# see--/speech_recognition

Measured on AMD Instinct MI355X. Metric: 1s 16kHz clips/sec training throughput, higher is better.
Workload: dtype f32; 1 GPU; configs[1]: 12-class conv_1d_time_sliced_with_attention, batch 1024/GPU synthetic 16000-sample fp32 clips, sampler+augment+STFT/mel(80,60)+raw fwd/bwd+RMSprop; global_batch=1024, parallelism=dp1, clip_bank=65536

## Files before the change

speech_recognition_amd/csrc/bn.hip:

```cpp
#include "internal.h"

namespace {

constexpr int FIN_CG = 16, FIN_RG = 16;
#ifndef KWS_FIN_U
#define KWS_FIN_U 16
#endif
constexpr int FIN_U = KWS_FIN_U;

__device__ float g_zero_fin[8] = {0.f, 0.f, 0.f, 0.f, 0.f, 0.f, 0.f, 0.f};

__global__ __launch_bounds__(256) void bn_stats_finalize_kernel(const float* __restrict__ part, int n_tiles,
                                                                double inv_count, int C,
                                                                const float* __restrict__ gamma,
                                                                const float* __restrict__ beta, float eps,
                                                                float one_minus_momentum, float* moving_mean,
                                                                float* moving_var, float* __restrict__ bn) {
  __shared__ double red[2][FIN_RG][FIN_CG];
  const int cg = threadIdx.x % FIN_CG, rg = threadIdx.x / FIN_CG;
  const int c = blockIdx.x * FIN_CG + cg;
  double s = 0.0, ss = 0.0;
  if (c < C) {
    for (int t = rg; t < n_tiles; t += FIN_U * FIN_RG) {
      float a[FIN_U], b[FIN_U];
// ... 22 lines not shown
      ss += red[1][r][cg];
    }
    const double mean = s * inv_count;
    double var = ss * inv_count - mean * mean;
    if (var < 0.0) var = 0.0;
    const float rstd = (float)(1.0 / sqrt(var + (double)eps));
    const float meanf = (float)mean, varf = (float)var;
    const float scale = gamma[c] * rstd;
    bn[c] = scale;
    bn[C + c] = beta[c] - meanf * scale;
    bn[2 * C + c] = meanf;
    bn[3 * C + c] = rstd;
    if (moving_mean) {
      moving_mean[c] = moving_mean[c] - (moving_mean[c] - meanf) * one_minus_momentum;
      moving_var[c] = moving_var[c] - (moving_var[c] - varf) * one_minus_momentum;
    }
  }
}

__global__ __launch_bounds__(256) void slice_reduce_kernel(const float* __restrict__ in, float* __restrict__ out,
                                                           int n, int W, int rows_per) {
  const int w = blockIdx.x * 256 + threadIdx.x;
  const int s = blockIdx.y;
  if (w >= W) return;
  const int r0 = s * rows_per;
  int r1 = r0 + rows_per;
  if (r1 > n) r1 = n;
  float a0 = 0.f, a1 = 0.f, a2 = 0.f, a3 = 0.f;
  int r = r0;
  for (; r + 3 < r1; r += 4) {
// ... 178 lines not shown
int pre_reduce(const float* part, int n, int W, float* scratch, hipStream_t st, const float** out_part, int* out_n) {
  if (scratch == nullptr || n <= KWS_PRE_REDUCE_MIN) {
    *out_part = part;
    *out_n = n;
    return KWS_OK;
  }
  const int rows_per = ceil_div(n, KWS_REDUCE_SLICES);
  const int S = ceil_div(n, rows_per);
  hipLaunchKernelGGL(slice_reduce_kernel, dim3((unsigned)ceil_div(W, 256), (unsigned)S), dim3(256), 0, st, part, scratch,
                     n, W, rows_per);
  KWS_LAUNCH_CHECK("slice_reduce_kernel");
  *out_part = scratch;
  *out_n = S;
  return KWS_OK;
}

}

int kws_dw_grad_finalize_batch(const float* const* part, const int* n_parts, const int* C, float* const* dw, int count,
                               hipStream_t stream) {
  KWS_REQUIRE(part && n_parts && C && dw && count > 0 && count <= KWS_DW_FIN_BATCH, "dw_grad_finalize_batch: bad arguments (count=%d)", count);
  DwFinBatch b;
  int blocks = 0;
  double bytes = 0;
  for (int i = 0; i < count; ++i) {
    KWS_REQUIRE(part[i] && dw[i] && n_parts[i] > 0 && n_parts[i] <= 8 * KWS_REDUCE_SLICES && C[i] > 0,
                "dw_grad_finalize_batch: bad entry %d (rows %d)", i, n_parts[i]);
    b.part[i] = part[i]; b.dw[i] = dw[i]; b.n_parts[i] = n_parts[i]; b.C[i] = C[i];
    blocks += ceil_div(C[i], FIN_CG);
    b.blk_end[i] = blocks;
// ... 7 lines not shown
}

extern "C" {

int kws_bn_stats_finalize(const float* stats_part, int n_tiles, int64_t count, int C, const float* gamma,
                          const float* beta, float eps, float momentum, float* moving_mean, float* moving_var,
                          float* bn, float* scratch, void* stream) {
  KWS_REQUIRE(stats_part && gamma && beta && bn, "bn_stats_finalize: NULL pointer");
  KWS_REQUIRE(n_tiles > 0 && count > 0 && C > 0, "bn_stats_finalize: bad sizes");
  KWS_REQUIRE((moving_mean == nullptr) == (moving_var == nullptr), "bn_stats_finalize: moving stats must both be set");
  const float omm = (float)(1.0 - (double)momentum);
  KwsProfScope prof("bn_finalize", 0.0, 8.0 * n_tiles * C, (hipStream_t)stream);
#ifdef KWS_ABL_NO_FIN
  return KWS_OK;
#endif
  KWS_TRY(pre_reduce(stats_part, n_tiles, 2 * C, scratch, (hipStream_t)stream, &stats_part, &n_tiles));
  hipLaunchKernelGGL(bn_stats_finalize_kernel, dim3((unsigned)ceil_div(C, FIN_CG)), dim3(FIN_CG * FIN_RG), 0, (hipStream_t)stream,
                     stats_part, n_tiles, 1.0 / (double)count, C, gamma, beta, eps, omm, moving_mean, moving_var, bn);
  KWS_LAUNCH_CHECK("bn_stats_finalize_kernel");
  return KWS_OK;
}

int kws_bn_infer_prepare(const float* gamma, const float* beta, const float* moving_mean, const float* moving_var,
                         float eps, int C, float* bn, void* stream) {
  KWS_REQUIRE(gamma && beta && moving_mean && moving_var && bn && C > 0, "bn_infer_prepare: bad arguments");
  hipLaunchKernelGGL(bn_infer_prepare_kernel, dim3((unsigned)ceil_div(C, 256)), dim3(256), 0, (hipStream_t)stream,
                     gamma, beta, moving_mean, moving_var, eps, C, bn);
  KWS_LAUNCH_CHECK("bn_infer_prepare_kernel");
  return KWS_OK;
}
// ... 59 lines not shown
```

speech_recognition_amd/csrc/conv1.hip:

```cpp
#include "internal.h"

#ifndef KWS_C1_WS
#define KWS_C1_WS 0
#endif
#ifndef KWS_C1_ABL
#define KWS_C1_ABL 0
#endif

namespace {

typedef float f32x16 __attribute__((ext_vector_type(16)));

constexpr int NOUT = 128;
constexpr int FM = 64;
constexpr int UM = 32;
#ifndef KWS_C1W_OCC
#define KWS_C1W_OCC 3
#endif
#ifndef KWS_C1W_ABL
#define KWS_C1W_ABL 0
#endif

struct Conv1Args {
  const float* x;
// ... 470 lines not shown
__global__ __launch_bounds__(256, KWS_C1W_OCC) void conv1_wgrad_slabsum_kernel(Conv1Args p, SlabBatch b, int n_conv) {
  __shared__ float sA[2][UM * KF];
  __shared__ float4 red[4][64];
  if ((int)blockIdx.x < n_conv) conv1_wgrad_body<KF>(p, sA, blockIdx.x);
  else kws_reduce_slabs_batch_body(b, (int)blockIdx.x - n_conv, red);
}

__global__ __launch_bounds__(256) void conv1_unfold_sum_kernel(const float* __restrict__ ws, float* __restrict__ dW,
                                                               int groups, int64_t group_stride, int taps, int cin, int hop) {
  const int i = blockIdx.x * 256 + threadIdx.x;
  if (i >= taps * cin * (NOUT / 4)) return;
  const int n4 = i % (NOUT / 4), jc = i / (NOUT / 4);
  const int j = jc / cin, c = jc - j * cin;
  const float4* src = reinterpret_cast<const float4*>(ws) + (int64_t)(hop * j + c) * (NOUT / 4) + n4;
  float4 s = make_float4(0.f, 0.f, 0.f, 0.f);
  for (int g = 0; g < groups; ++g) {
    const float4 v = src[(int64_t)g * group_stride];
    s.x += v.x; s.y += v.y; s.z += v.z; s.w += v.w;
  }
  reinterpret_cast<float4*>(dW)[i] = s;
}

struct WgradPlan {
  int S;
  int64_t chunk;
};
WgradPlan wgrad_plan(int64_t M) {
  WgradPlan pl;
  int64_t chunk = ceil_div64(ceil_div64(M, 256 * KWS_C1W_OCC), UM) * UM;
  if (chunk < UM) chunk = UM;
  pl.chunk = chunk;
  pl.S = (int)ceil_div64(M, chunk);
  return pl;
// ... 77 lines not shown
```

speech_recognition_amd/csrc/gemm.hip:

```cpp
#include "common.h"
#include "internal.h"

#include <algorithm>
#include <map>
#include <mutex>
#include <tuple>
#include <type_traits>

typedef float f32x16 __attribute__((ext_vector_type(16)));

#ifdef KWS_GEMM_STAMP
__device__ unsigned long long g_stamps[8192][8];
extern "C" __attribute__((visibility("default"))) int kws_debug_read_stamps(unsigned long long* out) {
  return (int)hipMemcpyFromSymbol(out, HIP_SYMBOL(g_stamps), sizeof(g_stamps));
}
#endif

namespace {

constexpr int NXCD = 8;

struct NNArgs {
  const float* A;
  const float* W;
// ... 1117 lines not shown
__global__ __launch_bounds__(256) void transpose_kernel(const float* in, float* out, int rows, int cols) {
  __shared__ float tile[32][33];
  const int bx = blockIdx.x * 32, by = blockIdx.y * 32;
  const int tx = threadIdx.x & 31, ty = threadIdx.x >> 5;
  for (int r = ty; r < 32; r += 8) {
    const int y = by + r, x = bx + tx;
    tile[r][tx] = (y < rows && x < cols) ? in[(int64_t)y * cols + x] : 0.f;
  }
  __syncthreads();
  for (int r = ty; r < 32; r += 8) {
    const int y = bx + r, x = by + tx;
    if (y < cols && x < rows) out[(int64_t)y * rows + x] = tile[tx][r];
  }
}

struct TransposeBatch {
  const float* in[KWS_TRANSPOSE_BATCH];
  float* out[KWS_TRANSPOSE_BATCH];
  int rows[KWS_TRANSPOSE_BATCH], cols[KWS_TRANSPOSE_BATCH], tile_end[KWS_TRANSPOSE_BATCH];
  int n;
};
__global__ __launch_bounds__(256) void transpose_batch_kernel(TransposeBatch b) {
  __shared__ float tile[32][33];
  int m = 0;
  while (m + 1 < b.n && (int)blockIdx.x >= b.tile_end[m]) ++m;
  const int t = blockIdx.x - (m ? b.tile_end[m - 1] : 0);
  const int rows = b.rows[m], cols = b.cols[m];
  const int tx_n = (cols + 31) / 32;
  const int bx = (t % tx_n) * 32, by = (t / tx_n) * 32;
  const float* in = b.in[m];
  float* out = b.out[m];
  const int tx = threadIdx.x & 31, ty = threadIdx.x >> 5;
  for (int r = ty; r < 32; r += 8) {
    const int y = by + r, x = bx + tx;
    tile[r][tx] = (y < rows && x < cols) ? in[(int64_t)y * cols + x] : 0.f;
  }
  __syncthreads();
  for (int r = ty; r < 32; r += 8) {
    const int y = bx + r, x = by + tx;
    if (y < cols && x < rows) out[(int64_t)y * rows + x] = tile[tx][r];
  }
}

__global__ __launch_bounds__(256) void reduce_slabs_batch_kernel(SlabBatch b) {
  __shared__ float4 red[4][64];
  kws_reduce_slabs_batch_body(b, blockIdx.x, red);
}

struct TNPlan {
  int bko, bno;
  int k_tiles, n_tiles, S;
  int64_t chunk;
};
bool tn_ws_eligible(int K, int N, bool gather) { return !gather && K % 64 == 0 && N % 64 == 0; }
#ifndef KWS_TN_MAX_S
#define KWS_TN_MAX_S 256
// ... 433 lines not shown
  const unsigned gx = (unsigned)ceil_div64(n4, 64);
  if (S > 128 && gx < 256) {
    const int per_group = 32, groups = ceil_div(S, per_group);
    hipLaunchKernelGGL(reduce_slabs_kernel, dim3(gx, (unsigned)groups), dim3(256), 0, st, ws, const_cast<float*>(ws), n4, S,
                       n4, per_group, (int64_t)per_group * n4);
    KWS_LAUNCH_CHECK("reduce_slabs_kernel");
    hipLaunchKernelGGL(reduce_slabs_kernel, dim3(gx), dim3(256), 0, st, ws, out, n4, groups, (int64_t)per_group * n4, 0,
                       (int64_t)0);
  } else {
    hipLaunchKernelGGL(reduce_slabs_kernel, dim3(gx), dim3(256), 0, st, ws, out, n4, S, (int64_t)-1, 0, (int64_t)0);
  }
  KWS_LAUNCH_CHECK("reduce_slabs_kernel");
  return KWS_OK;
}

int kws_transpose_batch_f32(const float* const* in, float* const* out, const int* rows, const int* cols, int n,
                            hipStream_t stream) {
  KWS_REQUIRE(in && out && rows && cols && n > 0 && n <= KWS_TRANSPOSE_BATCH, "transpose_batch: bad arguments (n=%d)", n);
  TransposeBatch b;
  int tiles = 0;
  double bytes = 0;
  for (int i = 0; i < n; ++i) {
    KWS_REQUIRE(in[i] && out[i] && rows[i] > 0 && cols[i] > 0, "transpose_batch: bad matrix %d", i);
    b.in[i] = in[i]; b.out[i] = out[i]; b.rows[i] = rows[i]; b.cols[i] = cols[i];
    tiles += ceil_div(rows[i], 32) * ceil_div(cols[i], 32);
    b.tile_end[i] = tiles;
    bytes += 8.0 * rows[i] * cols[i];
  }
  b.n = n;
  KwsProfScope prof("transpose", 0.0, bytes, stream);
  hipLaunchKernelGGL(transpose_batch_kernel, dim3((unsigned)tiles), dim3(256), 0, stream, b);
  KWS_LAUNCH_CHECK("transpose_batch_kernel");
  return KWS_OK;
}

}
```

speech_recognition_amd/csrc/internal.h:

```cpp
#pragma once
#include "common.h"

struct kws_ts_tail_args {
  const float* y; const float* bn; const float* W1; const float* b1; const float* W2; const float* labels;
  float* probs; float* g; float* part; float* xd; float* fd; float* dl1; float* dl2; float* per_loss;
  float* per_correct; float* att; int B, T, C, NC; uint64_t seed; uint32_t step; float keep_prob; float label_smoothing;
  int loss_batch; int64_t row_offset; int train;
};
int kws_ts_tail_launch(const kws_ts_tail_args* p, hipStream_t st);
constexpr int KWS_SMALL_WGRAD_SLICES = 32;
int kws_small_wgrad_launch(const float* X, const float* D, float* out, float* out_bias, int B, int K, int N,
                           float* scratch, hipStream_t st);
int kws_metrics_launch(const float* per_loss, const float* per_correct, int B, float* metrics, hipStream_t st);
struct kws_tail_post_args {
  const float* X2; const float* D2; float* ws2; int K2, N2;
  const float* X1; const float* D1; float* ws1; int K1, N1;
  float* bias1;
  const float* per_loss; const float* per_correct; float* metrics;
  int B;
};
int kws_tail_post_launch(const kws_tail_post_args* a, int* S_out, hipStream_t st);
bool kws_conv1_supported(const kws_gather_t* g, const kws_gather_t* unfolded, int N);
int kws_conv1_stats_rows(int64_t M);
int kws_conv1_fwd(const float* x, const kws_gather_t* g, const kws_gather_t* unfolded, const float* W, float* y, int B, int N,
                  float* stats, hipStream_t st);
int64_t kws_conv1_wgrad_workspace_floats(int64_t M);
int kws_conv1_wgrad(const float* x, const kws_gather_t* g, const kws_gather_t* unfolded, const float* G, float* dW, int B,
                    int N, float* workspace, hipStream_t st);
int kws_conv1_wgrad_slabs(const float* x, const kws_gather_t* g, const kws_gather_t* unfolded, const float* G, float* dW, int B,
                          int N, float* workspace, const float* const* sl_ws, float* const* sl_out, const int64_t* sl_n,
                          const int* sl_S, int n_sl, hipStream_t st);
extern "C" int kws_reduce_slab_groups_f32(float* ws, int64_t n, int S, int per_group, hipStream_t st);
extern "C" int kws_reduce_slabs_f32(const float* ws, float* out, int64_t n, int S, hipStream_t st);
extern "C" int kws_dwconv_bwd_acc_f32(const float* dz, const float* y, const float* w, const float* add, float* g, float* part,
                                      int B, int L_in, int L_out, int C, int stride, int pad_l, hipStream_t st);
extern "C" int kws_dwconv_bwd_acc_strided_f32(const float* dz, const float* y, const float* w, const float* add, int add_stride, int add_len,
// ... 44 lines not shown
int kws_gbn_bwd_finish(float* g, const float* y, const float* bn, int64_t M, const kws_gbn_cols* c, const float* part, int rows,
                       float* coef, float* dgamma0, int64_t pstride, int64_t boff, hipStream_t st);
struct kws_flat_tail_args {
  const float* y; const float* bn; int Ng;
  const float* Wd; const float* bd; const float* labels;
  float* probs; float* fd; float* dl; float* dA; float* per_loss; float* per_correct;
  int B, D, F, NC;
  uint64_t seed; uint32_t step; float keep_prob; int loss_batch; int64_t row_offset; uint32_t layer_id;
  int raw;
};
int kws_flat_tail_launch(const kws_flat_tail_args* a, int training, hipStream_t st);
int kws_pool3s2_same_fwd_pitch(const float* y, const float* bn, float* z, int zp, int B, int L, int C, hipStream_t st);
int kws_pool3s2_same_bwd_pitch(const float* dz, int zp, const float* y, const float* bn, float* g, float* part, int B, int L, int C,
                               hipStream_t st);
#ifdef __HIPCC__
__device__ __forceinline__ void kws_add4(float4& a, const float4 b) { a.x += b.x; a.y += b.y; a.z += b.z; a.w += b.w; }
__device__ __forceinline__ void kws_reduce_slabs_batch_body(const SlabBatch& b, int bid, float4 (*red)[64]) {
  int m = 0;
  while (m + 1 < b.n && bid >= b.blk_end[m]) ++m;
  const int t = bid - (m ? b.blk_end[m - 1] : 0);
  const int col = threadIdx.x & 63, grp = threadIdx.x >> 6;
  const int64_t n4 = b.n4[m];
  const int S = b.S[m];
  const int64_t i = (int64_t)t * 64 + col;
  const float4* w = reinterpret_cast<const float4*>(b.ws[m]);
  float4 s0 = make_float4(0.f, 0.f, 0.f, 0.f), s1 = s0, s2 = s0, s3 = s0;
  if (i < n4 && b.order[m]) {
    float4 t2 = s0;
    int k = grp;
    for (; k + 4 < S; k += 8) {
// ... 108 lines not shown
      used += need;
      ++count;
      return 0;
    }
    const int rc2 = kws_gemm_nn_f32(dY, WT, dZ, M, cout, cin, nullptr, st);
    if (rc2) return rc2;
    return gemm(Z, dY, dW, M, cin, cout, st);
  }
};
constexpr int KWS_DW_FIN_BATCH = 16;
int kws_dw_grad_finalize_batch(const float* const* part, const int* n_parts, const int* C, float* const* dw, int count,
                               hipStream_t stream);
constexpr int KWS_BN_INFER_BATCH = 16;
extern "C" int kws_bn_infer_prepare_batch(const float* const* gamma, const float* const* beta, const float* const* mm, const float* const* mv,
                               float eps, const int* C, float* const* bn, int count, hipStream_t stream);
constexpr int KWS_TRANSPOSE_BATCH = 16;
extern "C" int kws_transpose_batch_f32(const float* const* in, float* const* out, const int* rows, const int* cols, int n,
                                       hipStream_t stream);

struct kws_stft_plan {
  int frame_len, frame_step, fft_len, n_bins, n_mel, n_out;
  float log_offset, log_floor;
  int n_w;
  float* window;
  float2* w256;
  float2* w512;
  int* band_start;
  int* band_cnt;
  int* band_ofs;
  float* band_w;
  float* dct;
  float* dct64;
  float* b4;
// ... 14 lines not shown
```

speech_recognition_amd/csrc/net.hip:

```cpp
#include "net_internal.h"
#include <math.h>
#include <stdlib.h>

int64_t kws_net_add_tensor(kws_net* n, const std::string& name, std::vector<int64_t> shape, bool is_state, float l2,
                           int fan_in, int fan_out, float init) {
  kws_tensor_info_t t;
  memset(&t, 0, sizeof(t));
  snprintf(t.name, sizeof(t.name), "%s", name.c_str());
  int64_t size = 1;
  t.ndim = (int)shape.size();
  for (int i = 0; i < t.ndim; ++i) {
    t.shape[i] = shape[i];
    size *= shape[i];
  }
  t.size = size;
  t.is_state = is_state ? 1 : 0;
  t.l2 = l2;
  t.fan_in = fan_in;
  t.fan_out = fan_out;
  t.init = init;
  int64_t& cursor = is_state ? n->n_state : n->n_params;
  t.offset = cursor;
  cursor += (size + 3) / 4 * 4;
  n->tensors.push_back(t);
// ... 326 lines not shown
  float* red = ws + lo.red;
  const Dw3Run r{&lo.a, params, state, grads, ws, B, red, part, coef, DZ, st};
  const bool conv1_direct = kws_conv1_supported(&gather1f, &gather1, C1);
  const bool run_head = phase != 2;
  const int gmode = kws_net_get_gemm_mode(net);
  const bool h2 = gmode == 2;
  auto w_slots = [&](int i) { return slots(lo, ws, 0, i); };
  auto z_slots = [&](int i) { return slots(lo, ws, 1, i); };
  auto g_slots = [&](int i) { return slots(lo, ws, 2, i); };
  float* Gb[2] = {ws + lo.G, ws + lo.G2};
  KwsSlabQueue q;
  q.base = ws + lo.tns;
  q.cap = lo.tns_cap;
  q.allow_pair = gmode == 0;
  KWS_REQUIRE(nb + 2 <= KWS_SLAB_BATCH, "net: %d blocks exceed the slab batch", nb);
  if (run_head) {
    KWS_HIP(hipMemsetAsync(grads, 0, (size_t)net->n_params * 4, st));
    if (h2) KWS_TRY(split_kernels(lo, params, ws, true, st));
    {
      const int64_t M = (int64_t)B * lad.L1;
      const BnRef& bn1 = lad.bn1;
      if (conv1_direct) {
        KWS_TRY(kws_conv1_fwd(x, &gather1f, &gather1, params + conv1, r.y(0), B, C1, part, st));
      } else {
        KWS_TRY(fold_conv1(params, ws + lo.w1f, st));
        KWS_TRY(kws_gemm_gather_f32(x, &gather1f, ws + lo.w1f, r.y(0), B, C1, part, st));
      }
      const int rows1 = conv1_direct ? kws_conv1_stats_rows(M) : kws_gemm_gather_stats_rows(M);
      KWS_TRY(kws_bn_stats_finalize(part, rows1, M, C1, params + bn1.gamma, params + bn1.beta, KWS_BN_EPS, KWS_BN_MOMENTUM,
                                    state + bn1.mm, state + bn1.mv, r.bn_at(0), red, st));
    }
    KWS_TRY(blocks_fwd(lo, r, h2, part));
    kws_ts_tail_args t;
    memset(&t, 0, sizeof(t));
    t.y = r.y(nb); t.bn = r.bn_at(nb); t.W1 = params + d1k; t.b1 = params + d1b;
    t.W2 = params + d2k; t.labels = y_onehot; t.probs = probs; t.g = Gb[nb % 2]; t.part = part; t.xd = ws + lo.xd;
    t.fd = ws + lo.fd; t.dl1 = ws + lo.dl1; t.dl2 = ws + lo.dl2; t.per_loss = ws + lo.per_loss;
    t.per_correct = ws + lo.per_correct; t.att = ws + lo.att; t.B = B; t.T = T; t.C = C; t.NC = NC; t.seed = seed;
    t.step = step; t.keep_prob = DROP_KEEP; t.label_smoothing = LABEL_SMOOTH; t.loss_batch = loss_batch;
    t.row_offset = row_offset; t.train = 1;
    KWS_TRY(kws_ts_tail_launch(&t, st));
    bool tail_fused = false;
    if (gmode == 0) {
      kws_tail_post_args tp;
      tp.X2 = t.fd; tp.D2 = t.dl2; tp.ws2 = ws + lo.swg; tp.K2 = 2 * C; tp.N2 = NC;
      tp.X1 = t.xd; tp.D1 = t.dl1; tp.ws1 = ws + lo.swg1; tp.K1 = T * C; tp.N1 = T;
      tp.bias1 = grads + d1b; tp.per_loss = t.per_loss; tp.per_correct = t.per_correct; tp.metrics = metrics; tp.B = B;
      int S_tail = 0;
      const int rc = kws_tail_post_launch(&tp, &S_tail, st);
      if (rc < 0) return rc;
      tail_fused = rc == 0;
      if (tail_fused && S_tail > 0) {
        KWS_TRY(q.push(ws + lo.swg, grads + d2k, (int64_t)2 * C * NC, -S_tail, st));
        KWS_TRY(q.push(ws + lo.swg1, grads + d1k, (int64_t)T * C * T, -S_tail, st));
      }
    }
    if (!tail_fused) {
      KWS_TRY(kws_metrics_launch(t.per_loss, t.per_correct, B, metrics, st));
      KWS_TRY(kws_small_wgrad_launch(t.fd, t.dl2, grads + d2k, nullptr, B, 2 * C, NC, ws + lo.swg, st));
      KWS_TRY(kws_small_wgrad_launch(t.xd, t.dl1, grads + d1k, grads + d1b, B, T * C, T, ws + lo.swg, st));
    }
    const BnRef& last = lad.blocks[nb - 1].bn;
    KWS_TRY(kws_dw_bwd_finalize(part, B, (int64_t)B * T, last.C, nullptr, grads + last.gamma, grads + last.beta, coef, red, st));
    KWS_TRY(lad.transpose_all(r));
  }
  const int i_hi = phase == 2 ? split - 1 : nb - 1, i_lo = phase == 1 ? split : 0;
  for (int i = i_hi; i >= i_lo; --i) {
    const Dw3Block& b = lad.blocks[i];
    const int64_t M = (int64_t)B * b.Lout;
    float* Gcur = Gb[(i + 1) % 2];
    if (i == nb - 1)
      KWS_TRY(kws_bn_bwd_apply_amax(Gcur, r.y(i + 1), r.bn_at(i + 1), params + b.bn.gamma, coef, M, b.cout, h2 ? g_slots(i) : nullptr, st));
    if (!h2) {
      KWS_TRY(q.pair(Gcur, r.WT(i), DZ, r.z(i), grads + b.pw, M, b.cin, b.cout, st));
    } else {
      if (kws_gemm_nn_f16x2_supported(M, b.cout, b.cin))
        KWS_TRY(kws_gemm_nn_f16x2_f32(Gcur, ws + lo.WPd[i], DZ, M, b.cout, b.cin, g_slots(i), w_slots(i), nullptr, st));
      else
        KWS_TRY(kws_gemm_nn_f32(Gcur, r.WT(i), DZ, M, b.cout, b.cin, nullptr, st));
// ... 147 lines not shown
```

speech_recognition_amd/csrc/net_dw3ladder.hip:

```cpp
#include "net_internal.h"

int Dw3Ladder::build(KerasNames& kn, const int (*spec)[2], int n, int fm, int input_size) {
  int L = L1, cin = C1;
  for (int i = 0; i < n; ++i) {
    Dw3Block b;
    b.stride = spec[i][0];
    b.cin = cin;
    b.cout = spec[i][1] * fm;
    b.Lin = L;
    if (b.stride == 2) {
      kws_same_pad(L, 3, 2, &b.Lout, &b.pad_l);
    } else {
      b.Lout = L - 2;
      b.pad_l = 0;
    }
    KWS_REQUIRE(b.Lout >= 1, "net: input_size %d is too short: block %d keeps no row", input_size, i);
    b.dw = kn.dw(cin);
    b.pw = kn.conv(1, cin, b.cout, KWS_L2_COEF);
    b.bn = kn.bn(b.cout);
    blocks.push_back(b);
    L = b.Lout;
    cin = b.cout;
  }
  return KWS_OK;
// ... 60 lines not shown
  return KWS_OK;
}

int Dw3Ladder::infer_tables(const Dw3Run& r) const {
  KWS_REQUIRE(nb() + 1 <= KWS_BN_INFER_BATCH, "net: %d blocks exceed the BatchNorm table batch", nb());
  const float *ga[KWS_BN_INFER_BATCH], *be[KWS_BN_INFER_BATCH], *mm[KWS_BN_INFER_BATCH], *mv[KWS_BN_INFER_BATCH];
  float* tb[KWS_BN_INFER_BATCH];
  int Cs[KWS_BN_INFER_BATCH];
  for (int l = 0; l <= nb(); ++l) {
    const BnRef& b = l == 0 ? bn1 : blocks[l - 1].bn;
    ga[l] = r.params + b.gamma; be[l] = r.params + b.beta; mm[l] = r.state + b.mm; mv[l] = r.state + b.mv; tb[l] = r.bn_at(l); Cs[l] = b.C;
  }
  return kws_bn_infer_prepare_batch(ga, be, mm, mv, KWS_BN_EPS, Cs, tb, nb() + 1, r.st);
}

int Dw3Ladder::transpose_all(const Dw3Run& r) const {
  KWS_REQUIRE(nb() <= KWS_TRANSPOSE_BATCH, "net: %d blocks exceed the transpose batch", nb());
  const float* tin[KWS_TRANSPOSE_BATCH];
  float* tout[KWS_TRANSPOSE_BATCH];
  int trows[KWS_TRANSPOSE_BATCH], tcols[KWS_TRANSPOSE_BATCH];
  for (int i = 0; i < nb(); ++i) {
    tin[i] = r.params + blocks[i].pw; tout[i] = r.WT(i);
    trows[i] = blocks[i].cin; tcols[i] = blocks[i].cout;
  }
  return kws_transpose_batch_f32(tin, tout, trows, tcols, nb(), r.st);
}

int Dw3Ladder::fwd_dw(int i, const Dw3Run& r, unsigned* amax) const {
  const Dw3Block& b = blocks[i];
  return kws_dwconv_fwd_amax_f32(r.y(i), r.bn_at(i), r.params + b.dw, r.z(i), r.B, b.Lin, b.Lout, b.cin, b.stride, b.pad_l, amax, r.st);
}

int Dw3Ladder::stats_finalize(int i, const Dw3Run& r, const float* stats, int rows) const {
  const Dw3Block& b = blocks[i];
  return kws_bn_stats_finalize(stats, rows, (int64_t)r.B * b.Lout, b.cout, r.params + b.bn.gamma, r.params + b.bn.beta, KWS_BN_EPS,
                               KWS_BN_MOMENTUM, r.state + b.bn.mm, r.state + b.bn.mv, r.bn_at(i + 1), r.red, r.st);
}

int Dw3Ladder::fwd_block_f32(int i, const Dw3Run& r, float* stats, unsigned* amax) const {
  const Dw3Block& b = blocks[i];
  const int64_t M = (int64_t)r.B * b.Lout;
// ... 17 lines not shown
```

speech_recognition_amd/csrc/net_internal.h:

```cpp
#pragma once
#include <string.h>

#include <algorithm>
#include <atomic>
#include <memory>
#include <string>
#include <vector>

#include "internal.h"

constexpr float KWS_BN_EPS = 1e-3f;
constexpr float KWS_BN_MOMENTUM = 0.99f;
constexpr float KWS_L2_COEF = 1e-5f;

struct BnRef {
  int64_t gamma, beta;
  int64_t mm, mv;
  int C;
};
inline kws_gbn_refs kws_gbn_layer_refs(const BnRef& r, const float* params, float* state) {
  return kws_gbn_refs{params + r.gamma, 0, r.beta - r.gamma, state + r.mm, 0, r.mv - r.mm};
}
inline int kws_gbn_layer_bwd(float* dA, const float* y, const float* bn, const float* add, int64_t M, const kws_gbn_cols& c, float* part,
                             float* coef, float* grads, const BnRef& r, hipStream_t st) {
// ... 192 lines not shown
  float* bn_at(int l) const { return ws + o->bn + o->bn_stride * l; }
};
struct Dw3Ladder {
  int L1 = 0, C1 = 0;
  BnRef bn1;
  std::vector<Dw3Block> blocks;
  int nb() const { return (int)blocks.size(); }
  int build(KerasNames& kn, const int (*spec)[2], int n, int fm, int input_size);
  Dw3Sizes sizes(int B) const;
  void take_acts(Bump& bp, int B, bool training, const Dw3Sizes& s, Dw3Offsets* o) const;
  void take_bn(Bump& bp, int maxC, Dw3Offsets* o) const;
  void take_WT(Bump& bp, Dw3Offsets* o) const;
  int debug_view(const Dw3Offsets& o, int B, int what, int index, int64_t* offset_floats, int64_t* count) const;
  int infer_tables(const Dw3Run& r) const;
  int transpose_all(const Dw3Run& r) const;
  int fwd_dw(int i, const Dw3Run& r, unsigned* amax) const;
  int stats_finalize(int i, const Dw3Run& r, const float* stats, int rows) const;
  int fwd_block_f32(int i, const Dw3Run& r, float* stats, unsigned* amax) const;
  int bwd_block_input(int i, const Dw3Run& r, float* dy, unsigned* amax) const;
};

int kws_block_out_fwd(const float* y, const float* bn, const float* res, const float* res_bn, float* o, int B,
                      int L, int C, int pool, hipStream_t st);
int kws_block_out_dw_fwd(const float* y, const float* bn, const float* res, const float* res_bn, const float* w, float* o, float* z, int B,
                         int L, int C, int pool, hipStream_t st);
int kws_block_join_bwd_parts(int B, int L, int C, int pool);
int kws_block_join_bwd(const float* dO, const float* y, const float* bn, const float* gamma, const float* coef, float* out,
                       float* part, int pass, int B, int L, int C, int pool, int relu, hipStream_t st);
int64_t kws_block_out_bwd_part_floats(int B, int L, int C, int pool);
int kws_block_out_bwd(const float* dO, const float* y, const float* bn, float* g, float* part, int B, int L, int C,
// ... 49 lines not shown
```

speech_recognition_amd/csrc/tail.hip:

```cpp
#include "internal.h"

namespace {

constexpr int MAXT = 16;
constexpr int MAXNC = 64;

struct TailArgs {
  const float* y;
  const float* bn;
  const float* W1;
  const float* b1;
  const float* W2;
  const float* labels;
  float* probs;
  float* g;
  float* part;
  float* xd;
  float* fd;
  float* dl1;
  float* dl2;
  float* per_loss;
  float* per_correct;
  float* att_out;
  int B, T, C, NC;
// ... 517 lines not shown
  }
  if (threadIdx.x == 0) {
    metrics[0] = (float)rl[0];
    metrics[1] = rc[0];
    metrics[2] = 0.f;
    metrics[3] = 0.f;
  }
}
__global__ __launch_bounds__(256) void metrics_kernel(const float* per_loss, const float* per_correct, int B,
                                                      float* metrics) {
  metrics_body(per_loss, per_correct, B, metrics);
}

struct TailPost {
  kws_tail_post_args a;
  int rows_per, S, gx2, gx1;
};
__global__ __launch_bounds__(256) void tail_post_kernel(TailPost p) {
  int b = blockIdx.x;
  if (b < p.gx2 * p.S) {
    small_wgrad_rows_body<16>(p.a.X2, p.a.D2, p.a.ws2, p.a.B, p.a.K2, p.a.N2, p.rows_per, b % p.gx2, b / p.gx2);
    return;
  }
  b -= p.gx2 * p.S;
  if (b < p.gx1 * p.S) {
    small_wgrad_rows_body<16>(p.a.X1, p.a.D1, p.a.ws1, p.a.B, p.a.K1, p.a.N1, p.rows_per, b % p.gx1, b / p.gx1);
    return;
  }
  b -= p.gx1 * p.S;
  if (b == 0) metrics_body(p.a.per_loss, p.a.per_correct, p.a.B, p.a.metrics);
  else colsum_body<16, 256>(p.a.D1, p.a.bias1, p.a.B, p.a.N1);
}

}

int kws_ts_tail_launch(const kws_ts_tail_args* p, hipStream_t st) {
  KWS_REQUIRE(p->T > 0 && p->T <= MAXT && p->NC > 0 && p->NC <= MAXNC && p->C > 0, "ts_tail: bad shape T=%d NC=%d",
              p->T, p->NC);
  const int TC = p->T * p->C;
  const size_t lds_floats = (size_t)TC + 4 * p->C + 4 * MAXNC + 4 * MAXT + 3 * MAXNC + 256 + MAXNC + MAXT;
  KWS_REQUIRE(lds_floats * 4 <= 160 * 1024, "ts_tail: T*C=%d does not fit LDS", TC);
  TailArgs a{};
  a.y = p->y; a.bn = p->bn; a.W1 = p->W1; a.b1 = p->b1; a.W2 = p->W2; a.labels = p->labels; a.probs = p->probs;
  a.g = p->g; a.part = p->part; a.xd = p->xd; a.fd = p->fd; a.dl1 = p->dl1; a.dl2 = p->dl2;
  a.per_loss = p->per_loss; a.per_correct = p->per_correct; a.att_out = p->att;
  a.B = p->B; a.T = p->T; a.C = p->C; a.NC = p->NC;
// ... 46 lines not shown
      KWS_TRY(kws_reduce_slabs_f32(scratch, out, n, S, st));
    } else {
      hipLaunchKernelGGL(slab_sum_kernel, dim3((unsigned)ceil_div64(n, 256)), dim3(256), 0, st, scratch, out, n, S);
      KWS_LAUNCH_CHECK("slab_sum_kernel");
    }
  }
  if (out_bias) {
    if (N <= 16) hipLaunchKernelGGL((colsum_kernel<16, 256>), dim3(1), dim3(256), 0, st, D, out_bias, B, N);
    else if (N <= 32) hipLaunchKernelGGL((colsum_kernel<32, 1024>), dim3(1), dim3(1024), 0, st, D, out_bias, B, N);
    else hipLaunchKernelGGL((colsum_kernel<64, 1024>), dim3(1), dim3(1024), 0, st, D, out_bias, B, N);
    KWS_LAUNCH_CHECK("colsum_kernel");
  }
  return KWS_OK;
}

int kws_tail_post_launch(const kws_tail_post_args* a, int* S_out, hipStream_t st) {
  KWS_REQUIRE(a && S_out && a->X2 && a->D2 && a->ws2 && a->X1 && a->D1 && a->ws1 && a->per_loss && a->per_correct && a->metrics && a->B > 0,
              "tail_post: bad arguments");
  int S = KWS_SMALL_WGRAD_SLICES;
  if (S > a->B) S = a->B;
  const int rows_per = ceil_div(a->B, S);
  S = ceil_div(a->B, rows_per);
  if (S <= 1 || a->N1 > 16 || a->N2 > 16 || rows_per > KWS_SMALL_WGRAD_ROWS || ((int64_t)a->K1 * a->N1) % 4 != 0 ||
      ((int64_t)a->K2 * a->N2) % 4 != 0)
    return 1;
  TailPost p;
  p.a = *a; p.rows_per = rows_per; p.S = S; p.gx2 = ceil_div(a->K2, 256); p.gx1 = ceil_div(a->K1, 256);
  const int blocks = (p.gx2 + p.gx1) * S + 1 + (a->bias1 ? 1 : 0);
  KwsProfScope prof("small_wgrad", 2.0 * a->B * ((double)a->K1 * a->N1 + (double)a->K2 * a->N2),
                    4.0 * ((double)a->B * (a->K1 + a->K2 + a->N1 + a->N2) + (double)S * ((double)a->K1 * a->N1 + (double)a->K2 * a->N2)), st);
  hipLaunchKernelGGL(tail_post_kernel, dim3((unsigned)blocks), dim3(256), 0, st, p);
  KWS_LAUNCH_CHECK("tail_post_kernel");
  *S_out = S;
  return KWS_OK;
}

int kws_metrics_launch(const float* per_loss, const float* per_correct, int B, float* metrics, hipStream_t st) {
  hipLaunchKernelGGL(metrics_kernel, dim3(1), dim3(256), 0, st, per_loss, per_correct, B, metrics);
  KWS_LAUNCH_CHECK("metrics_kernel");
  return KWS_OK;
}
```

Measured before the change: 232,200 clips/s.

## Fuse transpose and gradient zeroing into tail-post kernel; single-pass sliced BN finalize

Moves the pointwise-weight transpose and the zeroing of padding gaps in the gradient buffer into the existing tail_post kernel as extra blocks. This drops the full-gradient hipMemsetAsync and a separate transpose launch when the fused path is taken. It also adds a BN stats finalize kernel that does the slice reduction and the final reduction in one launch, and unrolls the group sum in the conv1 wgrad reduction. The fused path relies on every gradient slot being fully overwritten except the padding gaps, which is a correctness risk if any gradient is accumulated rather than written.

```diff
diff --git a/speech_recognition_amd/csrc/bn.hip b/speech_recognition_amd/csrc/bn.hip
--- a/speech_recognition_amd/csrc/bn.hip
+++ b/speech_recognition_amd/csrc/bn.hip
@@ -60,6 +60,107 @@
     if (moving_mean) {
       moving_mean[c] = moving_mean[c] - (moving_mean[c] - meanf) * one_minus_momentum;
       moving_var[c] = moving_var[c] - (moving_var[c] - varf) * one_minus_momentum;
+    }
+  }
+}
+
+constexpr int FIN_SG = KWS_REDUCE_SLICES;
+constexpr int FIN_SLICED_MAX = 32 * KWS_REDUCE_SLICES;
+
+template <int Q, int QB>
+__device__ __forceinline__ void fin_slice_sums(const float* __restrict__ part, int n, int C, int rows_per, int c, int s,
+                                               float (&out)[Q]) {
+  const int r0 = s * rows_per < n ? s * rows_per : n;
+  const int r1 = r0 + rows_per < n ? r0 + rows_per : n;
+  const int nq = (r1 - r0) / 4, rr = r0 + 4 * nq;
+  float rem[3][Q];
+#pragma unroll
+  for (int u = 0; u < 3; ++u) {
+    const bool ok = rr + u < r1;
+    const float* src = ok ? part + (int64_t)(rr + u) * Q * C + c : g_zero_fin;
+#pragma unroll
+    for (int q = 0; q < Q; ++q) rem[u][q] = src[ok ? q * C : q];
+  }
+  float acc[Q][4];
+#pragma unroll
+  for (int q = 0; q < Q; ++q) acc[q][0] = acc[q][1] = acc[q][2] = acc[q][3] = 0.f;
+  for (int q0 = 0; q0 < nq; q0 += QB) {
+    float v[QB][4][Q];
+#pragma unroll
+    for (int j = 0; j < QB; ++j)
+#pragma unroll
+      for (int k = 0; k < 4; ++k) {
+        const bool ok = q0 + j < nq;
+        const float* src = ok ? part + (int64_t)(r0 + 4 * (q0 + j) + k) * Q * C + c : g_zero_fin;
+#pragma unroll
+        for (int q = 0; q < Q; ++q) v[j][k][q] = src[ok ? q * C : q];
+      }
+#pragma unroll
+    for (int j = 0; j < QB; ++j)
+#pragma unroll
+      for (int k = 0; k < 4; ++k)
+#pragma unroll
+        for (int q = 0; q < Q; ++q) acc[q][k] += v[j][k][q];
+  }
+#pragma unroll
+  for (int u = 0; u < 3; ++u)
+#pragma unroll
+    for (int q = 0; q < Q; ++q) acc[q][0] += rem[u][q];
+#pragma unroll
+  for (int q = 0; q < Q; ++q) out[q] = (acc[q][0] + acc[q][1]) + (acc[q][2] + acc[q][3]);
+}
+
+__global__ __launch_bounds__(FIN_CG * FIN_SG) void bn_stats_finalize_sliced_kernel(
+    const float* __restrict__ part, int n_tiles, int rows_per, float* __restrict__ slice_out, double inv_count, int C,
+    const float* __restrict__ gamma, const float* __restrict__ beta, float eps, float one_minus_momentum, float* moving_mean,
+    float* moving_var, float* __restrict__ bn) {
+  __shared__ double red[2][FIN_RG][FIN_CG];
+  __shared__ float sl[2][FIN_SG][FIN_CG];
+  const int cg = threadIdx.x % FIN_CG, sg = threadIdx.x / FIN_CG;
+  const int c = blockIdx.x * FIN_CG + cg;
+  const bool lead = sg == 0 && c < C;
+  const float ga = (lead ? gamma + c : g_zero_fin)[0], be = (lead ? beta + c : g_zero_fin)[0];
+  const float mm0 = (lead && moving_mean ? moving_mean + c : g_zero_fin)[0];
+  const float mv0 = (lead && moving_mean ? moving_var + c : g_zero_fin)[0];
+  const int S = (n_tiles + rows_per - 1) / rows_per;
+  float o[2] = {0.f, 0.f};
+  if (c < C) fin_slice_sums<2, 8>(part, n_tiles, C, rows_per, c, sg, o);
+  sl[0][sg][cg] = o[0];
+  sl[1][sg][cg] = o[1];
+  if (c < C && sg < S) {
+    slice_out[(int64_t)sg * 2 * C + c] = o[0];
+    slice_out[(int64_t)sg * 2 * C + C + c] = o[1];
+  }
+  __syncthreads();
+  if (sg < FIN_RG) {
+    double s = 0.0, ss = 0.0;
+    for (int t = sg; t < S; t += FIN_RG) {
+      s += (double)sl[0][t][cg];
+      ss += (double)sl[1][t][cg];
+    }
+    red[0][sg][cg] = s;
+    red[1][sg][cg] = ss;
+  }
+  __syncthreads();
+  if (lead) {
+    double s = 0.0, ss = 0.0;
+    for (int r = 0; r < FIN_RG; ++r) {
+      s += red[0][r][cg];
+      ss += red[1][r][cg];
+    }
+    const double mean = s * inv_count;
+    double var = ss * inv_count - mean * mean;
+    if (var < 0.0) var = 0.0;
+    const float rstd = (float)(1.0 / sqrt(var + (double)eps));
+    const float meanf = (float)mean, varf = (float)var;
+    const float scale = ga * rstd;
+    bn[c] = scale;
+    bn[C + c] = be - meanf * scale;
+    bn[2 * C + c] = meanf;
+    bn[3 * C + c] = rstd;
+    if (moving_mean) {
+      moving_mean[c] = mm0 - (mm0 - meanf) * one_minus_momentum;
+      moving_var[c] = mv0 - (mv0 - varf) * one_minus_momentum;
     }
   }
 }
@@ -268,6 +369,7 @@
   *out_n = S;
   return KWS_OK;
 }
+bool fin_sliced(const float* scratch, int n) { return scratch != nullptr && n > KWS_PRE_REDUCE_MIN && n <= FIN_SLICED_MAX; }
 
 }
 
@@ -305,6 +407,13 @@
 #ifdef KWS_ABL_NO_FIN
   return KWS_OK;
 #endif
+  if (fin_sliced(scratch, n_tiles)) {
+    hipLaunchKernelGGL(bn_stats_finalize_sliced_kernel, dim3((unsigned)ceil_div(C, FIN_CG)), dim3(FIN_CG * FIN_SG), 0, (hipStream_t)stream,
+                       stats_part, n_tiles, ceil_div(n_tiles, KWS_REDUCE_SLICES), scratch, 1.0 / (double)count, C, gamma, beta, eps, omm,
+                       moving_mean, moving_var, bn);
+    KWS_LAUNCH_CHECK("bn_stats_finalize_sliced_kernel");
+    return KWS_OK;
+  }
   KWS_TRY(pre_reduce(stats_part, n_tiles, 2 * C, scratch, (hipStream_t)stream, &stats_part, &n_tiles));
   hipLaunchKernelGGL(bn_stats_finalize_kernel, dim3((unsigned)ceil_div(C, FIN_CG)), dim3(FIN_CG * FIN_RG), 0, (hipStream_t)stream,
                      stats_part, n_tiles, 1.0 / (double)count, C, gamma, beta, eps, omm, moving_mean, moving_var, bn);
diff --git a/speech_recognition_amd/csrc/conv1.hip b/speech_recognition_amd/csrc/conv1.hip
--- a/speech_recognition_amd/csrc/conv1.hip
+++ b/speech_recognition_amd/csrc/conv1.hip
@@ -508,9 +508,15 @@
   const int j = jc / cin, c = jc - j * cin;
   const float4* src = reinterpret_cast<const float4*>(ws) + (int64_t)(hop * j + c) * (NOUT / 4) + n4;
   float4 s = make_float4(0.f, 0.f, 0.f, 0.f);
-  for (int g = 0; g < groups; ++g) {
-    const float4 v = src[(int64_t)g * group_stride];
-    s.x += v.x; s.y += v.y; s.z += v.z; s.w += v.w;
+  for (int g0 = 0; g0 < groups; g0 += 8) {
+    float4 v[8];
+#pragma unroll
+    for (int u = 0; u < 8; ++u) v[u] = src[(int64_t)(g0 + u < groups ? g0 + u : groups - 1) * group_stride];
+#pragma unroll
+    for (int u = 0; u < 8; ++u) {
+      const bool ok = g0 + u < groups;
+      s.x += ok ? v[u].x : 0.f; s.y += ok ? v[u].y : 0.f; s.z += ok ? v[u].z : 0.f; s.w += ok ? v[u].w : 0.f;
+    }
   }
   reinterpret_cast<float4*>(dW)[i] = s;
 }
diff --git a/speech_recognition_amd/csrc/gemm.hip b/speech_recognition_amd/csrc/gemm.hip
--- a/speech_recognition_amd/csrc/gemm.hip
+++ b/speech_recognition_amd/csrc/gemm.hip
@@ -1155,32 +1155,9 @@
   }
 }
 
-struct TransposeBatch {
-  const float* in[KWS_TRANSPOSE_BATCH];
-  float* out[KWS_TRANSPOSE_BATCH];
-  int rows[KWS_TRANSPOSE_BATCH], cols[KWS_TRANSPOSE_BATCH], tile_end[KWS_TRANSPOSE_BATCH];
-  int n;
-};
-__global__ __launch_bounds__(256) void transpose_batch_kernel(TransposeBatch b) {
+__global__ __launch_bounds__(256) void transpose_batch_kernel(KwsTransposeBatch b) {
   __shared__ float tile[32][33];
-  int m = 0;
-  while (m + 1 < b.n && (int)blockIdx.x >= b.tile_end[m]) ++m;
-  const int t = blockIdx.x - (m ? b.tile_end[m - 1] : 0);
-  const int rows = b.rows[m], cols = b.cols[m];
-  const int tx_n = (cols + 31) / 32;
-  const int bx = (t % tx_n) * 32, by = (t / tx_n) * 32;
-  const float* in = b.in[m];
-  float* out = b.out[m];
-  const int tx = threadIdx.x & 31, ty = threadIdx.x >> 5;
-  for (int r = ty; r < 32; r += 8) {
-    const int y = by + r, x = bx + tx;
-    tile[r][tx] = (y < rows && x < cols) ? in[(int64_t)y * cols + x] : 0.f;
-  }
-  __syncthreads();
-  for (int r = ty; r < 32; r += 8) {
-    const int y = bx + r, x = by + tx;
-    if (y < cols && x < rows) out[(int64_t)y * rows + x] = tile[tx][r];
-  }
+  kws_transpose_batch_body(b, (int)blockIdx.x, tile);
 }
 
 __global__ __launch_bounds__(256) void reduce_slabs_batch_kernel(SlabBatch b) {
@@ -1644,20 +1621,30 @@
   return KWS_OK;
 }
 
-int kws_transpose_batch_f32(const float* const* in, float* const* out, const int* rows, const int* cols, int n,
-                            hipStream_t stream) {
-  KWS_REQUIRE(in && out && rows && cols && n > 0 && n <= KWS_TRANSPOSE_BATCH, "transpose_batch: bad arguments (n=%d)", n);
-  TransposeBatch b;
+int kws_transpose_batch_fill(KwsTransposeBatch* b, const float* const* in, float* const* out, const int* rows, const int* cols, int n,
+                             int* tiles_out, double* bytes_out) {
+  KWS_REQUIRE(b && in && out && rows && cols && n > 0 && n <= KWS_TRANSPOSE_BATCH, "transpose_batch: bad arguments (n=%d)", n);
   int tiles = 0;
   double bytes = 0;
   for (int i = 0; i < n; ++i) {
     KWS_REQUIRE(in[i] && out[i] && rows[i] > 0 && cols[i] > 0, "transpose_batch: bad matrix %d", i);
-    b.in[i] = in[i]; b.out[i] = out[i]; b.rows[i] = rows[i]; b.cols[i] = cols[i];
+    b->in[i] = in[i]; b->out[i] = out[i]; b->rows[i] = rows[i]; b->cols[i] = cols[i];
     tiles += ceil_div(rows[i], 32) * ceil_div(cols[i], 32);
-    b.tile_end[i] = tiles;
+    b->tile_end[i] = tiles;
     bytes += 8.0 * rows[i] * cols[i];
   }
-  b.n = n;
+  b->n = n;
+  *tiles_out = tiles;
+  if (bytes_out) *bytes_out = bytes;
+  return KWS_OK;
+}
+
+int kws_transpose_batch_f32(const float* const* in, float* const* out, const int* rows, const int* cols, int n,
+                            hipStream_t stream) {
+  KwsTransposeBatch b;
+  int tiles = 0;
+  double bytes = 0;
+  KWS_TRY(kws_transpose_batch_fill(&b, in, out, rows, cols, n, &tiles, &bytes));
   KwsProfScope prof("transpose", 0.0, bytes, stream);
   hipLaunchKernelGGL(transpose_batch_kernel, dim3((unsigned)tiles), dim3(256), 0, stream, b);
   KWS_LAUNCH_CHECK("transpose_batch_kernel");
diff --git a/speech_recognition_amd/csrc/internal.h b/speech_recognition_amd/csrc/internal.h
--- a/speech_recognition_amd/csrc/internal.h
+++ b/speech_recognition_amd/csrc/internal.h
@@ -19,7 +19,28 @@
   const float* per_loss; const float* per_correct; float* metrics;
   int B;
 };
+constexpr int KWS_TRANSPOSE_BATCH = 16;
+struct KwsTransposeBatch {
+  const float* in[KWS_TRANSPOSE_BATCH];
+  float* out[KWS_TRANSPOSE_BATCH];
+  int rows[KWS_TRANSPOSE_BATCH], cols[KWS_TRANSPOSE_BATCH], tile_end[KWS_TRANSPOSE_BATCH];
+  int n;
+};
+extern "C" int kws_transpose_batch_fill(KwsTransposeBatch* b, const float* const* in, float* const* out, const int* rows, const int* cols,
+                                        int n, int* tiles_out, double* bytes_out);
+extern "C" int kws_transpose_batch_f32(const float* const* in, float* const* out, const int* rows, const int* cols, int n,
+                                       hipStream_t stream);
+constexpr int KWS_TAIL_ZERO_MAX = 8;
+struct kws_tail_riders {
+  KwsTransposeBatch tb;
+  int tiles;
+  float* zero[KWS_TAIL_ZERO_MAX];
+  int zero_cnt[KWS_TAIL_ZERO_MAX];
+  int n_zero;
+};
+bool kws_tail_post_takes(int B, int K1, int N1, int K2, int N2);
 int kws_tail_post_launch(const kws_tail_post_args* a, int* S_out, hipStream_t st);
+int kws_tail_post_riders_launch(const kws_tail_post_args* a, const kws_tail_riders* riders, int* S_out, hipStream_t st);
 bool kws_conv1_supported(const kws_gather_t* g, const kws_gather_t* unfolded, int N);
 int kws_conv1_stats_rows(int64_t M);
 int kws_conv1_fwd(const float* x, const kws_gather_t* g, const kws_gather_t* unfolded, const float* W, float* y, int B, int N,
@@ -94,6 +115,26 @@
 int kws_pool3s2_same_bwd_pitch(const float* dz, int zp, const float* y, const float* bn, float* g, float* part, int B, int L, int C,
                                hipStream_t st);
 #ifdef __HIPCC__
+__device__ __forceinline__ void kws_transpose_batch_body(const KwsTransposeBatch& b, int bid, float (*tile)[33]) {
+  int m = 0;
+  while (m + 1 < b.n && bid >= b.tile_end[m]) ++m;
+  const int t = bid - (m ? b.tile_end[m - 1] : 0);
+  const int rows = b.rows[m], cols = b.cols[m];
+  const int tx_n = (cols + 31) / 32;
+  const int bx = (t % tx_n) * 32, by = (t / tx_n) * 32;
+  const float* in = b.in[m];
+  float* out = b.out[m];
+  const int tx = threadIdx.x & 31, ty = threadIdx.x >> 5;
+  for (int r = ty; r < 32; r += 8) {
+    const int y = by + r, x = bx + tx;
+    tile[r][tx] = (y < rows && x < cols) ? in[(int64_t)y * cols + x] : 0.f;
+  }
+  __syncthreads();
+  for (int r = ty; r < 32; r += 8) {
+    const int y = bx + r, x = by + tx;
+    if (y < cols && x < rows) out[(int64_t)y * rows + x] = tile[tx][r];
+  }
+}
 __device__ __forceinline__ void kws_add4(float4& a, const float4 b) { a.x += b.x; a.y += b.y; a.z += b.z; a.w += b.w; }
 __device__ __forceinline__ void kws_reduce_slabs_batch_body(const SlabBatch& b, int bid, float4 (*red)[64]) {
   int m = 0;
@@ -232,9 +273,6 @@
 constexpr int KWS_BN_INFER_BATCH = 16;
 extern "C" int kws_bn_infer_prepare_batch(const float* const* gamma, const float* const* beta, const float* const* mm, const float* const* mv,
                                float eps, const int* C, float* const* bn, int count, hipStream_t stream);
-constexpr int KWS_TRANSPOSE_BATCH = 16;
-extern "C" int kws_transpose_batch_f32(const float* const* in, float* const* out, const int* rows, const int* cols, int n,
-                                       hipStream_t stream);
 
 struct kws_stft_plan {
   int frame_len, frame_step, fft_len, n_bins, n_mel, n_out;
diff --git a/speech_recognition_amd/csrc/net.hip b/speech_recognition_amd/csrc/net.hip
--- a/speech_recognition_amd/csrc/net.hip
+++ b/speech_recognition_amd/csrc/net.hip
@@ -364,8 +364,23 @@
   q.cap = lo.tns_cap;
   q.allow_pair = gmode == 0;
   KWS_REQUIRE(nb + 2 <= KWS_SLAB_BATCH, "net: %d blocks exceed the slab batch", nb);
+  kws_tail_riders riders;
+  memset(&riders, 0, sizeof(riders));
+  bool post_fused = run_head && gmode == 0 && kws_tail_post_takes(B, T * C, T, 2 * C, NC);
+  if (post_fused) {
+    for (const kws_tensor_info_t& ti : net->tensors) {
+      const int gap = (int)((4 - ti.size % 4) % 4);
+      if (ti.is_state || gap == 0) continue;
+      if (riders.n_zero == KWS_TAIL_ZERO_MAX) {
+        post_fused = false;
+        break;
+      }
+      riders.zero[riders.n_zero] = grads + ti.offset + ti.size;
+      riders.zero_cnt[riders.n_zero++] = gap;
+    }
+  }
   if (run_head) {
-    KWS_HIP(hipMemsetAsync(grads, 0, (size_t)net->n_params * 4, st));
+    if (!post_fused) KWS_HIP(hipMemsetAsync(grads, 0, (size_t)net->n_params * 4, st));
     if (h2) KWS_TRY(split_kernels(lo, params, ws, true, st));
     {
       const int64_t M = (int64_t)B * lad.L1;
@@ -390,17 +405,18 @@
     t.step = step; t.keep_prob = DROP_KEEP; t.label_smoothing = LABEL_SMOOTH; t.loss_batch = loss_batch;
     t.row_offset = row_offset; t.train = 1;
     KWS_TRY(kws_ts_tail_launch(&t, st));
-    bool tail_fused = false;
-    if (gmode == 0) {
+    const bool tail_fused = post_fused;
+    if (post_fused) {
       kws_tail_post_args tp;
       tp.X2 = t.fd; tp.D2 = t.dl2; tp.ws2 = ws + lo.swg; tp.K2 = 2 * C; tp.N2 = NC;
       tp.X1 = t.xd; tp.D1 = t.dl1; tp.ws1 = ws + lo.swg1; tp.K1 = T * C; tp.N1 = T;
       tp.bias1 = grads + d1b; tp.per_loss = t.per_loss; tp.per_correct = t.per_correct; tp.metrics = metrics; tp.B = B;
       int S_tail = 0;
-      const int rc = kws_tail_post_launch(&tp, &S_tail, st);
+      KWS_TRY(lad.transpose_batch(r, &riders.tb, &riders.tiles));
+      const int rc = kws_tail_post_riders_launch(&tp, &riders, &S_tail, st);
       if (rc < 0) return rc;
-      tail_fused = rc == 0;
-      if (tail_fused && S_tail > 0) {
+      KWS_REQUIRE(rc == 0, "net: tail_post declined a shape kws_tail_post_takes accepted");
+      if (S_tail > 0) {
         KWS_TRY(q.push(ws + lo.swg, grads + d2k, (int64_t)2 * C * NC, -S_tail, st));
         KWS_TRY(q.push(ws + lo.swg1, grads + d1k, (int64_t)T * C * T, -S_tail, st));
       }
@@ -412,7 +428,7 @@
     }
     const BnRef& last = lad.blocks[nb - 1].bn;
     KWS_TRY(kws_dw_bwd_finalize(part, B, (int64_t)B * T, last.C, nullptr, grads + last.gamma, grads + last.beta, coef, red, st));
-    KWS_TRY(lad.transpose_all(r));
+    if (!tail_fused) KWS_TRY(lad.transpose_all(r));
   }
   const int i_hi = phase == 2 ? split - 1 : nb - 1, i_lo = phase == 1 ? split : 0;
   for (int i = i_hi; i >= i_lo; --i) {
diff --git a/speech_recognition_amd/csrc/net_dw3ladder.hip b/speech_recognition_amd/csrc/net_dw3ladder.hip
--- a/speech_recognition_amd/csrc/net_dw3ladder.hip
+++ b/speech_recognition_amd/csrc/net_dw3ladder.hip
@@ -98,7 +98,7 @@
   return kws_bn_infer_prepare_batch(ga, be, mm, mv, KWS_BN_EPS, Cs, tb, nb() + 1, r.st);
 }
 
-int Dw3Ladder::transpose_all(const Dw3Run& r) const {
+int Dw3Ladder::transpose_batch(const Dw3Run& r, KwsTransposeBatch* tb, int* tiles) const {
   KWS_REQUIRE(nb() <= KWS_TRANSPOSE_BATCH, "net: %d blocks exceed the transpose batch", nb());
   const float* tin[KWS_TRANSPOSE_BATCH];
   float* tout[KWS_TRANSPOSE_BATCH];
@@ -107,8 +107,11 @@
     tin[i] = r.params + blocks[i].pw; tout[i] = r.WT(i);
     trows[i] = blocks[i].cin; tcols[i] = blocks[i].cout;
   }
+  if (tb) return kws_transpose_batch_fill(tb, tin, tout, trows, tcols, nb(), tiles, nullptr);
   return kws_transpose_batch_f32(tin, tout, trows, tcols, nb(), r.st);
 }
+
+int Dw3Ladder::transpose_all(const Dw3Run& r) const { return transpose_batch(r, nullptr, nullptr); }
 
 int Dw3Ladder::fwd_dw(int i, const Dw3Run& r, unsigned* amax) const {
   const Dw3Block& b = blocks[i];
diff --git a/speech_recognition_amd/csrc/net_internal.h b/speech_recognition_amd/csrc/net_internal.h
--- a/speech_recognition_amd/csrc/net_internal.h
+++ b/speech_recognition_amd/csrc/net_internal.h
@@ -230,6 +230,7 @@
   int debug_view(const Dw3Offsets& o, int B, int what, int index, int64_t* offset_floats, int64_t* count) const;
   int infer_tables(const Dw3Run& r) const;
   int transpose_all(const Dw3Run& r) const;
+  int transpose_batch(const Dw3Run& r, KwsTransposeBatch* tb, int* tiles) const;
   int fwd_dw(int i, const Dw3Run& r, unsigned* amax) const;
   int stats_finalize(int i, const Dw3Run& r, const float* stats, int rows) const;
   int fwd_block_f32(int i, const Dw3Run& r, float* stats, unsigned* amax) const;
diff --git a/speech_recognition_amd/csrc/tail.hip b/speech_recognition_amd/csrc/tail.hip
--- a/speech_recognition_amd/csrc/tail.hip
+++ b/speech_recognition_amd/csrc/tail.hip
@@ -555,9 +555,11 @@
 
 struct TailPost {
   kws_tail_post_args a;
-  int rows_per, S, gx2, gx1;
+  int rows_per, S, gx2, gx1, n_bias;
+  kws_tail_riders r;
 };
 __global__ __launch_bounds__(256) void tail_post_kernel(TailPost p) {
+  __shared__ float tile[32][33];
   int b = blockIdx.x;
   if (b < p.gx2 * p.S) {
     small_wgrad_rows_body<16>(p.a.X2, p.a.D2, p.a.ws2, p.a.B, p.a.K2, p.a.N2, p.rows_per, b % p.gx2, b / p.gx2);
@@ -569,8 +571,18 @@
     return;
   }
   b -= p.gx1 * p.S;
-  if (b == 0) metrics_body(p.a.per_loss, p.a.per_correct, p.a.B, p.a.metrics);
-  else colsum_body<16, 256>(p.a.D1, p.a.bias1, p.a.B, p.a.N1);
+  if (b == 0) {
+    metrics_body(p.a.per_loss, p.a.per_correct, p.a.B, p.a.metrics);
+    const int z = threadIdx.x / 4, k = threadIdx.x % 4;
+    if (z < p.r.n_zero && k < p.r.zero_cnt[z]) p.r.zero[z][k] = 0.f;
+    return;
+  }
+  b -= 1;
+  if (b < p.n_bias) {
+    colsum_body<16, 256>(p.a.D1, p.a.bias1, p.a.B, p.a.N1);
+    return;
+  }
+  kws_transpose_batch_body(p.r.tb, b - p.n_bias, tile);
 }
 
 }
@@ -647,19 +659,39 @@
   return KWS_OK;
 }
 
-int kws_tail_post_launch(const kws_tail_post_args* a, int* S_out, hipStream_t st) {
+static bool tail_post_plan(int B, int K1, int N1, int K2, int N2, int* S_out, int* rows_per_out) {
+  int S = KWS_SMALL_WGRAD_SLICES;
+  if (S > B) S = B;
+  const int rows_per = ceil_div(B, S);
+  S = ceil_div(B, rows_per);
+  *S_out = S;
+  *rows_per_out = rows_per;
+  return !(S <= 1 || N1 > 16 || N2 > 16 || rows_per > KWS_SMALL_WGRAD_ROWS || ((int64_t)K1 * N1) % 4 != 0 || ((int64_t)K2 * N2) % 4 != 0);
+}
+bool kws_tail_post_takes(int B, int K1, int N1, int K2, int N2) {
+  int S, rows_per;
+  return B > 0 && tail_post_plan(B, K1, N1, K2, N2, &S, &rows_per);
+}
+
+int kws_tail_post_launch(const kws_tail_post_args* a, int* S_out, hipStream_t st) { return kws_tail_post_riders_launch(a, nullptr, S_out, st); }
+
+int kws_tail_post_riders_launch(const kws_tail_post_args* a, const kws_tail_riders* riders, int* S_out, hipStream_t st) {
   KWS_REQUIRE(a && S_out && a->X2 && a->D2 && a->ws2 && a->X1 && a->D1 && a->ws1 && a->per_loss && a->per_correct && a->metrics && a->B > 0,
               "tail_post: bad arguments");
-  int S = KWS_SMALL_WGRAD_SLICES;
-  if (S > a->B) S = a->B;
-  const int rows_per = ceil_div(a->B, S);
-  S = ceil_div(a->B, rows_per);
-  if (S <= 1 || a->N1 > 16 || a->N2 > 16 || rows_per > KWS_SMALL_WGRAD_ROWS || ((int64_t)a->K1 * a->N1) % 4 != 0 ||
-      ((int64_t)a->K2 * a->N2) % 4 != 0)
-    return 1;
+  KWS_REQUIRE(!riders || (riders->tiles >= 0 && riders->n_zero >= 0 && riders->n_zero <= KWS_TAIL_ZERO_MAX), "tail_post: bad riders");
+  int S, rows_per;
+  if (!tail_post_plan(a->B, a->K1, a->N1, a->K2, a->N2, &S, &rows_per)) return 1;
   TailPost p;
   p.a = *a; p.rows_per = rows_per; p.S = S; p.gx2 = ceil_div(a->K2, 256); p.gx1 = ceil_div(a->K1, 256);
-  const int blocks = (p.gx2 + p.gx1) * S + 1 + (a->bias1 ? 1 : 0);
+  p.n_bias = a->bias1 ? 1 : 0;
+  if (riders) {
+    p.r = *riders;
+    for (int i = 0; i < p.r.n_zero; ++i)
+      KWS_REQUIRE(p.r.zero[i] && p.r.zero_cnt[i] > 0 && p.r.zero_cnt[i] < 4, "tail_post: bad zero run %d", i);
+  } else {
+    p.r = kws_tail_riders{};
+  }
+  const int blocks = (p.gx2 + p.gx1) * S + 1 + p.n_bias + p.r.tiles;
   KwsProfScope prof("small_wgrad", 2.0 * a->B * ((double)a->K1 * a->N1 + (double)a->K2 * a->N2),
                     4.0 * ((double)a->B * (a->K1 + a->K2 + a->N1 + a->N2) + (double)S * ((double)a->K1 * a->N1 + (double)a->K2 * a->N2)), st);
   hipLaunchKernelGGL(tail_post_kernel, dim3((unsigned)blocks), dim3(256), 0, st, p);
```

After: 233,200 clips/s (median of 6 runs). About the same (+0.4%).
